# AndreiBarsan/DynSLAM

Measured on AMD Instinct MI355X. Metric: frames/sec TSDF integrate+raycast (KITTI 1242x375, 5mm voxels); HBM GB/s vs peak, higher is better.
Workload: dtype f32; 1 GPU; configs[1]: static map only, synthetic KITTI-like street 1242x375, preset 5mm (voxel 0.005 m, mu 0.02 m), frames 5..2062 of a 2063-frame sequence, one volume per GPU; visible_blocks_last_frame=122661, allocated_blocks=8388608, status=3, decay=False, swap=False, instances=0

## Files before the change

dynslam_amd/csrc/dsr_engine.hip:

```cpp
#include <sched.h>

#include "dsr_internal.h"
#include "dsr_math.h"
using namespace dsr_internal;
#include "k_alloc.h"
#include "k_composite.h"
#include "k_decay.h"
#include "k_integrate.h"
#include "k_raycast.h"
#include "k_swap.h"
#include "k_small.h"
#include "k_batch.h"
#include "k_batch_gc.h"
#include "../../include/dsr_track.h"
#include "../../include/dsr_gc.h"

extern "C" {
int dsri_batch_flush(dsr_batch *b);
bool dsri_batch_is_live(dsr_batch *b);
void dsri_batch_drop_deferred(dsr_batch *b);
}

namespace dsr_internal {
std::atomic<int> g_enginesOnDevice[64];
// ... 122 lines not shown
  F(e->scene.swapState); F(e->scene.swapStored); F(e->swapStagingDev); F(e->swapIdsDev); F(e->swapFlagsDev);
  F(e->scene.swapSlot); F(e->scene.hostSlabs);
  if (e->hostUsedSeen) (void)hipHostFree(e->hostUsedSeen);
  if (e->hostUsedEvent) (void)hipEventDestroy(e->hostUsedEvent);
  for (auto p : e->hostSlabs) (void)hipHostFree(p);
  for (int k = 0; k < 2; ++k) {
    if (e->upPin[k]) (void)hipHostFree(e->upPin[k]);
    if (e->upSlotFree[k]) (void)hipEventDestroy(e->upSlotFree[k]);
  }
  F(e->upDev); F(e->pvDev); F(e->xferRgb); F(e->xferDepth);
  F(e->rgbAlt); F(e->depthAlt);
  for (hipEvent_t ev : {e->evAltFree, e->evFusionRead}) if (ev) (void)hipEventDestroy(ev);
  if (e->viewStream && e->ownsViewStream) (void)hipStreamDestroy(e->viewStream);
  if (e->pvPin) (void)hipHostFree(e->pvPin);
  if (e->statusHost) (void)hipHostFree(e->statusHost);
  for (hipEvent_t ev : {e->evUploaded, e->evIngested, e->evView, e->evViewRead}) if (ev) (void)hipEventDestroy(ev);
  if (e->xEvent) (void)hipEventDestroy(e->xEvent);
  if (e->xEvent2) (void)hipEventDestroy(e->xEvent2);
  if (e->orderEvent) (void)hipEventDestroy(e->orderEvent);
  for (auto &p : e->profPending) { (void)hipEventDestroy(p.a); (void)hipEventDestroy(p.b); }
  for (auto ev : e->eventPool) (void)hipEventDestroy(ev);
  if (e->evList) (void)hipEventDestroy(e->evList);
  if (e->evExpected) (void)hipEventDestroy(e->evExpected);
  if (e->sideStream) (void)hipStreamDestroy(e->sideStream);
  if (e->stream && e->ownsStream) (void)hipStreamDestroy(e->stream);
}

int expected_depths(dsr_engine *e, RenderStateDev &rs, const FrameP &p);

int allocate_scene(dsr_engine *e) {
  e->sceneVersion++;
  e->noVisibleValid = false;
  e->listVersion++;
  float proj[4]; depth_proj(e, proj);
  FrameP p = make_frame_params(e, e->M_d, e->invM_d, proj);
  RenderStateDev &rs = e->live;
  { int st = before_fusion(e); if (st) return st; }
  if (e->sidePending) { HIP_TRY(hipStreamWaitEvent(e->stream, e->evExpected, 0)); e->sidePending = false; }
  if (e->smallPath) {
    const int tx0 = e->viewBox[0] / 16, ty0 = e->viewBox[1] / 16;
    const int tx1 = div_up(std::min(e->viewBox[2], e->W), 16), ty1 = div_up(std::min(e->viewBox[3], e->H), 16);
    if (tx1 > tx0 && ty1 > ty0)
      LAUNCH(e, "alloc_mark", k_alloc_mark<true>, dim3(tx1 - tx0, ty1 - ty0), dim3(256), p, e->scene, (const float *)e->depth,
             rs.visType, tx0, ty0);
    if (e->statusDev) e->statusSeq++;
    {
      ProfScope _ps(e, "small_alloc_visible");
      hipLaunchKernelGGL(k_small_alloc_visible, dim3(1), dim3(kSmallThreads), e->smallLdsBytes, e->stream, p, e->scene,
                         (const float *)e->depth, rs.visType, e->numTilesE, e->allocWork, rs.visibleIDs, rs.visBlocks, e->noBlocks,
                         e->statusDev, e->statusSeq, reinterpret_cast<int2 *>(rs.minmax), rs.rayBox, e->smallLists ? 1 : 0);
    }
    HIP_TRY(hipGetLastError());
    { int st = after_fusion(e); if (st) return st; }
    e->liveExp.valid = true; e->liveExp.onSide = false; e->liveExp.version = e->listVersion; e->liveExp.M = e->M_d;
    memcpy(e->liveExp.proj, proj, sizeof proj);
    return DSR_OK;
  }
  LAUNCH(e, "retest_prev_visible", k_retest_previous_visible, dim3(1024), dim3(256), p, e->scene,
         (const int4 *)rs.visBlocks, rs.visType);
  int2 *allocTile = reinterpret_cast<int2 *>(e->scene.allocTile);
  LAUNCH(e, "alloc_mark", k_alloc_mark<false>, dim3(div_up(e->W, 16), div_up(e->H, 16)), dim3(256), p, e->scene,
         (const float *)e->depth, rs.visType, 0, 0);
  LAUNCH(e, "scan_tiles", k_scan_tile_sums, dim3(1), dim3(1024), allocTile, e->numTilesE, e->scene, (int)SCAN_ALLOC, 0);
  LAUNCH(e, "alloc_commit", k_alloc_commit, dim3(e->numTilesE), dim3(kTileThreads), p, e->scene, allocTile, e->allocWork);
  LAUNCH(e, "alloc_apply", k_alloc_apply, dim3(256), dim3(256), p, e->scene, (const float *)e->depth,
         (const int4 *)e->allocWork, rs.visType);
  LAUNCH(e, "visible_count", k_visible_count<false>, dim3(e->numTilesE), dim3(kTileThreads), p, e->scene, rs.visType, e->tileSums);
  LAUNCH(e, "scan_tiles", k_scan_tile_sums, dim3(1), dim3(1024), e->tileSums, e->numTilesE, e->scene,
         (int)SCAN_VISIBLE_LIVE, e->noBlocks);
  if (e->statusDev) e->statusSeq++;
  LAUNCH(e, "visible_write", k_visible_write, dim3(e->numTilesE), dim3(kTileThreads), e->E, (const uint8_t *)rs.visType,
         (const int2 *)e->tileSums, rs.visibleIDs, e->noBlocks, e->scene, (int)e->s.use_swapping, rs.visBlocks, e->statusDev,
         e->statusSeq);
  HIP_TRY(hipGetLastError());
  { int st = after_fusion(e); if (st) return st; }
  e->liveExp.valid = false;
  if (e->overlapExpected && (e->device >= 64 || g_enginesOnDevice[e->device].load(std::memory_order_relaxed) <= 1)) {
    HIP_TRY(hipEventRecord(e->evList, e->stream));
    HIP_TRY(hipStreamWaitEvent(e->sideStream, e->evList, 0));
    {
      StreamSwap sw(e, e->sideStream);
      int st = expected_depths(e, rs, p);
      if (st) return st;
    }
    HIP_TRY(hipEventRecord(e->evExpected, e->sideStream));
    e->sidePending = true;
    e->liveExp.valid = true; e->liveExp.onSide = true; e->liveExp.version = e->listVersion; e->liveExp.M = e->M_d;
// ... 56 lines not shown
bool pair_render_default() {
  static const bool on = !(getenv("DSR_PAIR_RENDER") && atoi(getenv("DSR_PAIR_RENDER")) == 0);
  return on;
}
int launch_icp_maps(dsr_engine *e, const FrameP &p) {
  RenderStateDev &rs = e->live;
  dim3 g(div_up(e->W, 16), div_up(e->H, 16));
  if (rs.rayBox) LAUNCH(e, "icp_maps", k_icp_maps_box, g, dim3(256), p, e->scene, (const float4 *)rs.raycastResult, e->pointsMap,
                        e->normalsMap, rs.raycastImage, (const int32_t *)rs.rayBox);
  else LAUNCH(e, "icp_maps", k_icp_maps, g, dim3(256), p, e->scene, (const float4 *)rs.raycastResult, e->pointsMap,
              e->normalsMap, rs.raycastImage);
  return DSR_OK;
}
int flush_track_render(dsr_engine *e) {
  if (!e->trackRender.pending) return DSR_OK;
  e->trackRender.pending = false;
  int st = launch_raycast(e, "raycast", e->trackRender.p, e->live);
  if (st) return st;
  if ((st = launch_icp_maps(e, e->trackRender.p))) return st;
  HIP_TRY(hipGetLastError());
  return DSR_OK;
}

const char *status_text(int status) {
  return status == DSR_E_OUT_OF_BLOCKS ? "out of voxel blocks / excess list entries"
                                       : "allocation ray longer than the order key allows: the pose is not rigid (k_alloc.h)";
}

int sticky_status(dsr_engine *e, int *status) {
  static_assert(CTR_NO_VISIBLE_LIVE + 2 == CTR_STATUS, "the three words are fetched with one copy");
  int32_t w[3] = {0, 0, 0};
  HIP_TRY(hipMemcpyAsync(w, e->scene.ctr + CTR_NO_VISIBLE_LIVE, sizeof w, hipMemcpyDeviceToHost, e->stream));
  HIP_TRY(hipStreamSynchronize(e->stream));
  *status = w[2];
  e->noVisibleSeen = w[0]; e->noVisibleValid = true;
  return DSR_OK;
}

int published_status(dsr_engine *e, int *status) {
  if (!e->statusHost) return sticky_status(e, status);
  const int seq = e->statusSeq;
  for (unsigned spins = 1;; ++spins) {
    if ((int)((unsigned)__atomic_load_n(e->statusHost + 2, __ATOMIC_ACQUIRE) - (unsigned)seq) >= 0) break;
    if ((spins & 0xfff) == 0) {
      const hipError_t q = hipStreamQuery(e->stream);
      if (q == hipSuccess) {
// ... 75 lines not shown
  LAUNCH(e, "scan_tiles", k_scan_tile_sums, dim3(1), dim3(1024), e->tileSums, e->numTilesE, e->scene, (int)SCAN_SWAP_OUT,
         (int)kTransferBlocks);
  LAUNCH(e, "swap_list", (k_swap_write<true>), dim3(e->numTilesE), dim3(kTileThreads), e->scene, e->E,
         (const uint8_t *)e->live.visType, (const int2 *)e->tileSums, e->swapIdsDev, e->swapFlagsDev);
  LAUNCH(e, "swapout_move", k_swapout_move, dim3(1024), dim3(256), e->scene, (const int32_t *)e->swapIdsDev);
  e->hostUsedUpper += kTransferBlocks;
  e->hostUsedCallsSince++;
  if (!e->hostUsedPending) {
    HIP_TRY(hipMemcpyAsync(e->hostUsedSeen, e->scene.ctr + CTR_HOST_USED, 4, hipMemcpyDeviceToHost, e->stream));
    HIP_TRY(hipEventRecord(e->hostUsedEvent, e->stream));
    e->hostUsedPending = true;
    e->hostUsedCallsSince = 0;
  }
  HIP_TRY(hipGetLastError());
  return DSR_OK;
}

}

std::string &dsr_internal::last_error() {
  thread_local std::string message;
  return message;
}
int dsr_internal::engine_set_device(dsr_engine *e) { return set_device(e); }
void dsr_internal::prof_resolve_pending(dsr_engine *e) { prof_resolve(e); }
int dsr_internal::engine_flush_deferred(dsr_engine *e) {
  int st = flush_track_render(e);
  if (st) return st;
  if (e->ownerBatch) {
    if (dsri_batch_is_live(e->ownerBatch)) return dsri_batch_flush(e->ownerBatch);
    e->ownerBatch = nullptr;
  }
  return DSR_OK;
}
void dsr_internal::engine_prof_resolve(dsr_engine *e) { prof_resolve(e); }
int dsr_internal::engine_reset(dsr_engine *e) { return reset_scene(e); }
void dsr_internal::engine_list_entries(dsr_engine *e, const char *label, bool owning, const SceneP &sc, int2 *tileSums, int32_t *out,
                                       int capacity, int lengthCtr) {
  const int scanMode = lengthCtr == CTR_NO_ALLOCATED ? SCAN_ALLOCATED : SCAN_NCAND;
  if (owning) LAUNCH(e, label, k_owning_count, dim3(e->numTilesE), dim3(kTileThreads), sc, e->E, tileSums);
  else LAUNCH(e, label, k_allocated_count, dim3(e->numTilesE), dim3(kTileThreads), sc, e->E, tileSums);
  LAUNCH(e, "scan_tiles", k_scan_tile_sums, dim3(1), dim3(1024), tileSums, e->numTilesE, sc, scanMode, capacity);
  if (owning) LAUNCH(e, label, k_owning_write, dim3(e->numTilesE), dim3(kTileThreads), sc, e->E, (const int2 *)tileSums, out, capacity);
  else LAUNCH(e, label, k_allocated_write, dim3(e->numTilesE), dim3(kTileThreads), sc, e->E, (const int2 *)tileSums, out, capacity);
}
void dsr_internal::engine_scan_counts(dsr_engine *e, const SceneP &sc, const uint32_t *counts, const int32_t *nPtr, int n, int2 *tileSums,
                                      uint32_t *offsets) {
// ... 89 lines not shown

  int st = set_device(e);
  if (st) { delete e; return st; }
#define ALLOC(expr) if ((st = (expr)) != DSR_OK) { free_all(e); delete e; return st; }
  if (s.view_pipeline < DSR_VIEW_PIPELINE_AUTO || s.view_pipeline > DSR_VIEW_PIPELINE_SHARED) { delete e; return fail(DSR_E_ARG, "bad view_pipeline"); }
  const int pvMode = s.view_pipeline == DSR_VIEW_PIPELINE_OFF ? 0 : s.view_pipeline == DSR_VIEW_PIPELINE_PER_ENGINE ? 1
                     : s.view_pipeline == DSR_VIEW_PIPELINE_SHARED ? 3
                     : getenv("DSR_PIPELINED_VIEW") ? atoi(getenv("DSR_PIPELINED_VIEW")) : (s.sync_status ? 3 : 0);
  auto shared_stream = [&](hipStream_t *table) -> hipStream_t {
    if (e->device < 0 || e->device >= 64) return nullptr;
    std::lock_guard<std::mutex> lock(g_ioMutex);
    if (!table[e->device] && create_stream(&table[e->device]) != hipSuccess) table[e->device] = nullptr;
    return table[e->device];
  };
  if (pvMode == 3 && s.sdf_local_block_num <= 16384 && (e->stream = shared_stream(g_sharedViewStream))) e->ownsStream = false;
  else if (pvMode >= 2 && s.sdf_local_block_num <= 16384 && (e->stream = shared_stream(g_sharedSmallStream))) e->ownsStream = false;
  else if (create_stream(&e->stream) != hipSuccess) { delete e; return fail(DSR_E_DEVICE, "hipStreamCreate failed"); }
  e->overlapExpected = s.sdf_local_block_num >= (1 << 20);
  if (const char *ov = getenv("DSR_OVERLAP_EXPECTED")) e->overlapExpected = atoi(ov) != 0;
  if (e->overlapExpected &&
      (hipStreamCreateWithFlags(&e->sideStream, hipStreamNonBlocking) != hipSuccess ||
       hipEventCreateWithFlags(&e->evList, order_event_flags()) != hipSuccess ||
       hipEventCreateWithFlags(&e->evExpected, order_event_flags()) != hipSuccess)) { free_all(e); delete e; return fail(DSR_E_DEVICE, "side stream creation failed"); }
  ALLOC(dmalloc(&e->scene.table, (size_t)e->E));
  ALLOC(dmalloc(&e->scene.vba, (size_t)e->noBlocks * kBlockBytes));
  ALLOC(dmalloc(&e->scene.voxelAllocList, (size_t)e->noBlocks));
  ALLOC(dmalloc(&e->scene.excessAllocList, (size_t)e->noExcess));
  ALLOC(dmalloc(&e->scene.ctr, (size_t)CTR_COUNT));
  ALLOC(dmalloc(&e->scene.work, (size_t)WORK_COUNT));
  ALLOC(dmalloc(&e->scene.allocKey, (size_t)e->E));
  ALLOC(dmalloc(&e->scene.allocGrp, (size_t)e->numTilesE * (kTile / 32)));
  ALLOC(dmalloc(&e->scene.allocTile, (size_t)e->numTilesE + 1));
  {
    const int cells = ((e->W + 7) / 8) * ((e->H + 7) / 8);
    e->smallPath = e->smallVolume && !s.use_swapping && e->E <= kSmallMaxEntries && e->E % 8 == 0 && e->numTilesE <= kSmallMaxTiles &&
                   small_lds_bytes(cells) <= 64 * 1024;
    if (e->smallPath) {
      ALLOC(dmalloc(&e->scene.visGrp, (size_t)kSmallBitWords * 4));
      ALLOC(dmalloc(&e->scene.visBits, (size_t)kSmallBitWords));
      ALLOC(dmalloc(&e->scene.allocBits, (size_t)kSmallBitWords));
      ALLOC(dmalloc(&e->scene.allocIds, (size_t)e->noBlocks));
      e->smallLdsBytes = small_lds_bytes(cells);
      const size_t withLists = std::max(e->smallLdsBytes, sizeof(SmallShared) + small_lists_lds_bytes(e->noBlocks));
      e->smallLists = withLists <= 64 * 1024 && !(getenv("DSR_SMALL_LISTS") && atoi(getenv("DSR_SMALL_LISTS")) == 0);
      if (e->smallLists) e->smallLdsBytes = withLists;
      e->pairRender = pair_render_default();
// ... 182 lines not shown
  Mat4 M; memcpy(M.m, m, sizeof M.m);
  Mat4 inv;
  if (!m4_inv(M, inv)) return fail(DSR_E_ARG, "singular pose");
  e->M_d = M; e->invM_d = inv;
  return DSR_OK;
}
int dsr_get_pose(dsr_engine *e, float m_out[16], float inv_m_out[16]) {
  if (!e) return fail(DSR_E_ARG, "null");
  if (m_out) memcpy(m_out, e->M_d.m, sizeof e->M_d.m);
  if (inv_m_out) memcpy(inv_m_out, e->invM_d.m, sizeof e->invM_d.m);
  return DSR_OK;
}


int dsr_set_fusion_weight_params(dsr_engine *e, int depth_weighting) {
  if (!e) return fail(DSR_E_ARG, "null");
  e->depthWeighting = depth_weighting ? 1 : 0;
  return DSR_OK;
}

int dsr_allocate_scene_from_depth(dsr_engine *e) {
  CHECK_E(e);
  if (!e->hasView) return fail(DSR_E_NO_VIEW, "no view yet");
  int st = allocate_scene(e);
  if (st) return st;
  if (e->s.sync_status) {
    int status = DSR_OK;
    st = published_status(e, &status);
    if (st) return st;
    if (status != DSR_OK) return fail(status, status_text(status));
  }
  return DSR_OK;
}

int dsr_integrate_into_scene(dsr_engine *e) {
  CHECK_E(e);
  if (!e->hasView) return fail(DSR_E_NO_VIEW, "no view yet");
  return integrate_scene(e);
}

int dsr_process_frame(dsr_engine *e) {
  CHECK_E(e);
  if (!e->hasView) return fail(DSR_E_NO_VIEW, "no view yet");
  int st = allocate_scene(e);
  if (st) return st;
  st = integrate_scene(e);
  if (st) return st;
  if (e->s.use_swapping) {
    if ((st = swap_in(e))) return st;
    if ((st = swap_out(e))) return st;
  }
  e->framesProcessed++;
  if (e->s.sync_status) {
    int status = DSR_OK;
    st = published_status(e, &status);
    if (st) return st;
    if (status != DSR_OK) {
      (void)hipMemsetAsync(e->scene.ctr + CTR_STATUS, 0, 4, e->stream);
      if (e->statusHost) e->statusHost[1] = DSR_OK;
      return fail(status, status_text(status));
    }
  }
  return DSR_OK;
}

int dsr_prepare(dsr_engine *e) {
  CHECK_E(e);
  if (!e->hasView) return fail(DSR_E_NO_VIEW, "no view yet");
  float proj[4]; depth_proj(e, proj);
  FrameP p = make_frame_params(e, e->M_d, e->invM_d, proj);
  RenderStateDev &rs = e->live;
  if (e->liveExp.valid && e->liveExp.version == e->listVersion && memcmp(e->liveExp.M.m, e->M_d.m, sizeof e->M_d.m) == 0 &&
      memcmp(e->liveExp.proj, proj, sizeof proj) == 0) {
    if (e->liveExp.onSide) {
      HIP_TRY(hipStreamWaitEvent(e->stream, e->evExpected, 0));
      e->sidePending = false;
    }
  } else {
    if (e->sidePending) { HIP_TRY(hipStreamWaitEvent(e->stream, e->evExpected, 0)); e->sidePending = false; }
    e->liveExp.valid = false;
    int st = expected_depths(e, rs, p);
    if (st) return st;
  }
  if (e->pairRender && rs.rayBox) {
    e->trackRender.pending = true;
    e->trackRender.p = p;
    HIP_TRY(hipGetLastError());
    return DSR_OK;
  }
  {
// ... 201 lines not shown
                  float *depth_out) {
  CHECK_E_NOFLUSH(e);
  return render_common(e, type, pose_m, intrinsics, rgba_out, depth_out, false);
}

int dsr_get_image_dev(dsr_engine *e, int type, const float pose_m[16], const float intrinsics[4], void *rgba_out_dev,
                      void *depth_out_dev) {
  CHECK_E_NOFLUSH(e);
  return render_common(e, type, pose_m, intrinsics, rgba_out_dev, depth_out_dev, true);
}

int dsr_engine_share_stream(dsr_engine *e, dsr_engine *owner) {
  CHECK_E(e);
  if (!owner || owner == e) return fail(DSR_E_ARG, "bad stream owner");
  if (owner->device != e->device) return fail(DSR_E_ARG, "engines on different GPUs cannot share a stream");
  if (e->pipelinedView || owner->pipelinedView) return fail(DSR_E_ARG, "not with pipelined views (they have streams of their own)");
  HIP_TRY(hipStreamSynchronize(e->stream));
  if (e->sideStream) HIP_TRY(hipStreamSynchronize(e->sideStream));
  if (e->ownsStream && e->stream) (void)hipStreamDestroy(e->stream);
  e->stream = owner->stream;
  e->ownsStream = false;
  e->borrowedStream = true;
  e->overlapExpected = false;
  e->liveExp.valid = false;
  return DSR_OK;
}


struct dsr_batch {
  dsr_engine *source = nullptr;
  int device = 0;
  std::vector<dsr_engine *> vols;
  std::vector<BatchVolP> volsHost;
  BatchVolP *volsDev = nullptr;
  bool pair = false, pendingTrack = false;
  BatchFrames liveFrames;
  BatchFrameP *freeTableDev = nullptr;
  BatchTrackerDev *tracker = nullptr;
};
namespace {
std::mutex g_batchMutex;
std::vector<dsr_batch *> g_liveBatches;
}
bool dsri_batch_is_live(dsr_batch *b) {
  std::lock_guard<std::mutex> lock(g_batchMutex);
  return std::find(g_liveBatches.begin(), g_liveBatches.end(), b) != g_liveBatches.end();
// ... 373 lines not shown

int dsr_gc_debug_alloc_list(dsr_engine *e, int32_t *ids_out, int32_t capacity, int32_t *n, int32_t *valid) {
  CHECK_E(e);
  if (!n || !valid || capacity < 0 || (capacity > 0 && !ids_out)) return fail(DSR_E_ARG, "bad arguments");
  if (!e->scene.allocIds || !e->smallLists) return fail(DSR_E_ARG, "this engine keeps no sorted list of allocated entries");
  int32_t c[2] = {0, 0};
  HIP_TRY(hipMemcpyAsync(c, e->scene.ctr + CTR_NO_ALLOC_IDS, sizeof c, hipMemcpyDeviceToHost, e->stream));
  HIP_TRY(hipStreamSynchronize(e->stream));
  *n = c[0]; *valid = c[1];
  const int m = std::min(std::min(c[0], capacity), e->noBlocks);
  if (m > 0) {
    HIP_TRY(hipMemcpyAsync(ids_out, e->scene.allocIds, (size_t)m * 4, hipMemcpyDeviceToHost, e->stream));
    HIP_TRY(hipStreamSynchronize(e->stream));
  }
  return DSR_OK;
}

int dsr_gc_debug_fifo(dsr_engine *e, int32_t out[3]) {
  if (!e || !out) return fail(DSR_E_ARG, "bad arguments");
  out[0] = e->fifoHead; out[1] = e->fifoLen; out[2] = e->fifoCap;
  return DSR_OK;
}

int dsr_dump_swap_state(dsr_engine *e, uint8_t *states, uint8_t *has_stored) {
  CHECK_E(e);
  if (!e->scene.swapState) return fail(DSR_E_ARG, "swapping is not enabled");
  if (states) HIP_TRY(hipMemcpyAsync(states, e->scene.swapState, (size_t)e->E, hipMemcpyDeviceToHost, e->stream));
  if (has_stored) HIP_TRY(hipMemcpyAsync(has_stored, e->scene.swapStored, (size_t)e->E, hipMemcpyDeviceToHost, e->stream));
  HIP_TRY(hipStreamSynchronize(e->stream));
  return DSR_OK;
}

int dsr_dump_stored_block(dsr_engine *e, int entry, dsr_voxel *out, int *present) {
  CHECK_E(e);
  if (!present || entry < 0 || entry >= e->E) return fail(DSR_E_ARG, "bad entry");
  *present = 0;
  if (!e->scene.swapState) return DSR_OK;
  uint8_t flag = 0;
  HIP_TRY(hipMemcpy(&flag, e->scene.swapStored + entry, 1, hipMemcpyDeviceToHost));
  if (!flag) return DSR_OK;
  HIP_TRY(hipStreamSynchronize(e->stream));
  int32_t slot = -1;
  HIP_TRY(hipMemcpy(&slot, e->scene.swapSlot + entry, 4, hipMemcpyDeviceToHost));
  if (slot < 0 || slot >= (long long)e->hostSlabs.size() * e->scene.slabBlocks) return fail(DSR_E_DEVICE, "host store inconsistent");
  *present = 1;
  if (out) {
// ... 149 lines not shown
```

dynslam_amd/csrc/dsr_internal.h:

```cpp
#pragma once
#include <hip/hip_runtime.h>

#include <algorithm>
#include <atomic>
#include <cmath>
#include <cstdio>
#include <cstdlib>
#include <cstring>
#include <map>
#include <mutex>
#include <new>
#include <string>
#include <unordered_map>
#include <vector>

#include "dsr_device.h"
#include "dsr_insert.h"
#include "../../include/dsr_mesh.h"
#include "../../include/dsr_track.h"

using namespace dsr;

struct dsr_dense_grid;
struct dsr_erase_params;
// ... 20 lines not shown
struct RenderStateDev {
  int32_t *visibleIDs = nullptr;
  int32_t *visibleIDsAlt = nullptr;
  int4 *visBlocks = nullptr;
  int4 *visBlocksAlt = nullptr;
  uint8_t *visType = nullptr;
  float2 *minmax = nullptr;
  float4 *raycastResult = nullptr;
  uchar4 *raycastImage = nullptr;
  int32_t *rayBox = nullptr;
  int ctrIdx = CTR_NO_VISIBLE_LIVE;
};

struct ProfRec { std::string name; double ms = 0; long long launches = 0; };

struct dsr_engine {
  dsr_settings s;
  dsr_calib calib;
  int device = 0;
  hipStream_t stream = nullptr;
  hipStream_t sideStream = nullptr;
  hipEvent_t evList = nullptr, evExpected = nullptr;
  bool overlapExpected = true;
  unsigned long long listVersion = 0;
  struct { bool valid = false; bool onSide = false; unsigned long long version = 0; Mat4 M; float proj[4] = {0, 0, 0, 0}; } liveExp;
  int W = 0, H = 0, Wr = 0, Hr = 0, P = 0;
  int noBuckets = 0, noExcess = 0, E = 0, noBlocks = 0;
  int numTilesE = 0, numTilesB = 0, numTilesMax = 0;
  uint32_t maxSteps = 0;
  int gridPersistent = 2048;
  int gridDecay = 2048;
  int gridIntegrate = 8192;
  bool smallVolume = false;
  bool smallPath = false;
  bool smallLists = false;
  size_t smallLdsBytes = 0;
  int viewBox[4] = {0, 0, 0, 0};
  int blankBox[4] = {0, 0, 0, 0};
  bool blankValid = false;
  int gridExpected = 128;
  Mat4 calibInv, M_d, invM_d;

  SceneP scene{};
  RenderStateDev live, freeview;
  int2 *tileSums = nullptr;
  uint2 *integrateStats = nullptr;
// ... 150 lines not shown
extern std::mutex g_ioMutex;
extern hipStream_t g_ioStream[64];
hipError_t create_stream(hipStream_t *out);
int io_stream(dsr_engine *e, hipStream_t *out);
unsigned order_event_flags();
int make_event(hipEvent_t *ev, bool hostWaits = false);
int before_view_write(dsr_engine *e, hipStream_t stream);
int view_written(dsr_engine *e, hipStream_t stream);
int begin_view_modify(dsr_engine *e);
int before_fusion(dsr_engine *e);
int after_fusion(dsr_engine *e);
hipStream_t vstream(dsr_engine *e);
void cutout_write_region(const dsr_engine *instance, bool direct, int x0, int y0, int w, int h, int wr[4]);
void cutout_written(dsr_engine *instance, bool direct, int x0, int y0, int w, int h);
void tracker_free(dsr_engine *e);
struct BatchTrackerDev;
int batch_track_check(const dsr_track_settings *settings);
int batch_track(dsr_engine *src, dsr_engine *const *vols, int n, const dsr_track_settings *settings, BatchTrackerDev **bt,
                dsr_track_result *out);
void batch_tracker_free(BatchTrackerDev *bt);
extern std::atomic<int> g_enginesOnDevice[64];
int engine_set_device(dsr_engine *e);
int engine_flush_deferred(dsr_engine *e);
void engine_prof_resolve(dsr_engine *e);
void engine_list_entries(dsr_engine *e, const char *label, bool owning, const SceneP &sc, int2 *tileSums, int32_t *out, int capacity,
                         int lengthCtr = CTR_DECAY_NCAND);
void engine_free_flagged(dsr_engine *e, const int32_t *cand, const int32_t *nCandPtr);
void engine_scan_counts(dsr_engine *e, const SceneP &sc, const uint32_t *counts, const int32_t *nPtr, int n, int2 *tileSums,
                        uint32_t *offsets);
int engine_reset(dsr_engine *e);
int engine_ensure_fifo(dsr_engine *e, int slots);
int engine_add_host_slab(dsr_engine *e);
int engine_small_bit_words();
bool engine_in_live_batch(dsr_engine *e);
int engine_render(dsr_engine *e, int type, const float pose_m[16], const float intrinsics[4], void *rgba_out, void *depth_out,
                  bool outIsDevice);
int mesh_release(dsr_engine *e);
int dense_grid_check(dsr_engine *e, const dsr_dense_grid *grid, const char *what, bool importFields, dsr::DenseP &g, long long &n);
int erase_mask_check(const dsr_engine *e, const dsr_dense_grid *grid, const void *mask, const dsr_erase_params *params);
bool host_range_pinned(const void *p, size_t bytes);
int short_division_exact(hipStream_t stream, float b, bool *exact);
struct Scratch {
  const char *what;
  std::vector<void *> ptrs;
  hipStream_t stream = nullptr;
  bool ordered = false;
// ... 34 lines not shown
  unsigned long long *keysA, *keysB, *voxels;
  uint32_t *bucketsA, *bucketsB;
  int32_t *info, *exc, *excRank, *consumes, *blockRank, *res, *nUnique;
  int2 *plan;
  uint8_t *tmp;
  size_t tmpBytes = 0;
  explicit InsertScratch(const char *what) : sc(what) {}
  int init(int N, bool withSort, hipStream_t stream);
};
int ordered_insert(dsr_engine *dst, const dsr::MergeP &m, int N, const InsertScratch &s);
int ordered_insert(dsr_engine *dst, int N, const InsertScratch &s);
struct InsertOutcome { int32_t res[MR_COUNT]; unsigned long long voxels; int dropped; };
int insert_read_back(dsr_engine *e, const InsertScratch &s, InsertOutcome &o);
inline int two_volume_check(const dsr_engine *dst, const dsr_engine *src, const float *m, const char *what, const char *mName) {
  const std::string w(what);
  if (!dst || !src || !m) return fail(DSR_E_ARG, w + ": null argument");
  if (dst == src) return fail(DSR_E_ARG, w + ": dst and src are the same engine");
  if (dst->device != src->device) return fail(DSR_E_ARG, w + ": the engines sit on different devices (move one with dsr_snapshot_export / _import)");
  if (dst->s.use_swapping || src->s.use_swapping) return fail(DSR_E_ARG, w + ": engines with use_swapping are not supported");
  if (!rigid_transform(m)) return fail(DSR_E_ARG, w + ": " + mName + " is not a rigid transform");
  return DSR_OK;
}
}
using dsr_internal::host_range_pinned;
using dsr_internal::short_division_exact;

#define LAUNCH(e, name, kernel, grid, block, ...)                                \
  do {                                                                           \
    dsr_internal::ProfScope _ps((e), (name));                                    \
    hipLaunchKernelGGL(kernel, grid, block, 0, (e)->stream, __VA_ARGS__);        \
  } while (0)

#define CHECK_E_NOFLUSH(e)                                  \
  if (!(e)) return fail(DSR_E_ARG, "null engine");          \
  { int _st = dsr_internal::engine_set_device(e); if (_st) return _st; }
#define CHECK_E(e)                                          \
  CHECK_E_NOFLUSH(e)                                        \
  if ((e)->trackRender.pending || (e)->ownerBatch) { int _st = dsr_internal::engine_flush_deferred(e); if (_st) return _st; }
```

dynslam_amd/csrc/dsr_view.hip:

```cpp
#include "dsr_internal.h"
#include "k_edges.h"

using namespace dsr_internal;

namespace dsr_internal {
std::mutex g_ioMutex;
hipStream_t g_ioStream[64] = {};
}

namespace dsr_internal {


hipError_t create_stream(hipStream_t *out) { return hipStreamCreateWithFlags(out, hipStreamNonBlocking); }

int io_stream(dsr_engine *e, hipStream_t *out) {
  if (e->device < 0 || e->device >= 64) return fail(DSR_E_ARG, "device ordinal beyond the I/O stream table");
  std::lock_guard<std::mutex> lock(g_ioMutex);
  if (!g_ioStream[e->device]) HIP_TRY(create_stream(&g_ioStream[e->device]));
  *out = g_ioStream[e->device];
  return DSR_OK;
}

unsigned order_event_flags() { return hipEventDisableTiming | hipEventReleaseToDevice; }
int make_event(hipEvent_t *ev, bool hostWaits) {
// ... 16 lines not shown
  HIP_TRY(hipEventRecord(e->evView, stream));
  e->viewEventValid = true;
  return DSR_OK;
}
int io_reads_view(dsr_engine *e, hipStream_t io) {
  if (!e->viewEventValid) {
    int st = make_event(&e->evView, true);
    if (st) return st;
    HIP_TRY(hipEventRecord(e->evView, e->stream));
    e->viewEventValid = true;
  }
  HIP_TRY(hipStreamWaitEvent(io, e->evView, 0));
  return DSR_OK;
}
int io_read_done(dsr_engine *e, hipStream_t io) {
  int st = make_event(&e->evViewRead, true);
  if (st) return st;
  HIP_TRY(hipEventRecord(e->evViewRead, io));
  e->viewReadEver = true;
  return DSR_OK;
}

hipStream_t vstream(dsr_engine *e) { return e->pipelinedView ? e->viewStream : e->stream; }

void cutout_write_region(const dsr_engine *instance, bool direct, int x0, int y0, int w, int h, int wr[4]) {
  const int W = instance->W, H = instance->H;
  wr[0] = 0; wr[1] = 0; wr[2] = W; wr[3] = H;
  if (!direct || !instance->blankValid) return;
  const int b[4] = {std::max(0, x0), std::max(0, y0), std::min(W, x0 + w), std::min(H, y0 + h)};
  const int *o = instance->blankBox;
  const bool bEmpty = b[0] >= b[2] || b[1] >= b[3], oEmpty = o[0] >= o[2] || o[1] >= o[3];
  if (bEmpty && oEmpty) { wr[2] = 0; wr[3] = 0; return; }
  if (bEmpty) { for (int k = 0; k < 4; ++k) wr[k] = o[k]; return; }
  if (oEmpty) { for (int k = 0; k < 4; ++k) wr[k] = b[k]; return; }
  wr[0] = std::min(b[0], o[0]); wr[1] = std::min(b[1], o[1]); wr[2] = std::max(b[2], o[2]); wr[3] = std::max(b[3], o[3]);
}
void cutout_written(dsr_engine *instance, bool direct, int x0, int y0, int w, int h) {
  instance->blankValid = direct;
  instance->blankBox[0] = std::max(0, x0); instance->blankBox[1] = std::max(0, y0);
  instance->blankBox[2] = std::min(instance->W, x0 + w); instance->blankBox[3] = std::min(instance->H, y0 + h);
}

struct ViewTarget { uchar4 *rgb; float *depth; };

int begin_view_replace(dsr_engine *e, hipStream_t ws, ViewTarget *t) {
  int st = before_view_write(e, ws);
// ... 70 lines not shown
  HIP_TRY(hipStreamWaitEvent(consumer, e->evUploaded, 0));
  *cDev = e->upDev;
  *dDev = e->upDev + e->upDepthOff;
  return DSR_OK;
}
int upload_consumed(dsr_engine *e, hipStream_t consumer) {
  HIP_TRY(hipEventRecord(e->evIngested, consumer));
  e->ingestPending = true;
  return DSR_OK;
}

int filter_view(dsr_engine *e, float *depth) {
  if (!e->s.use_bilateral_filter) return DSR_OK;
  HIP_TRY(hipMemcpyAsync(e->depthTmp, depth, (size_t)e->P * 4, hipMemcpyDeviceToDevice, e->stream));
  dim3 g(div_up(e->W, 16), div_up(e->H, 16));
  for (int k = 0; k < 5; ++k) {
    if (k & 1) LAUNCH(e, "filter_depth", k_filter_depth, g, dim3(256), (const float *)e->depthTmp, depth, e->W, e->H);
    else LAUNCH(e, "filter_depth", k_filter_depth, g, dim3(256), (const float *)depth, e->depthTmp, e->W, e->H);
  }
  HIP_TRY(hipMemcpyAsync(depth, e->depthTmp, (size_t)e->P * 4, hipMemcpyDeviceToDevice, e->stream));
  return DSR_OK;
}

int convert_view(dsr_engine *e, const void *rgbDev, const void *depthDev, bool uploaded = false) {
  const float a = e->calib.disparity_calib[0], b = e->calib.disparity_calib[1];
  const size_t rgbBytes = (size_t)e->Wr * e->Hr * 4;
  hipStream_t ws = vstream(e);
  ViewTarget t;
  int st = begin_view_replace(e, ws, &t);
  if (st) return st;
  {
    StreamSwap sw(e, ws);
    if (((uintptr_t)rgbDev & 15) == 0 && ((uintptr_t)depthDev & 15) == 0) {
      const int nRgbVec = (int)(rgbBytes / 16), nQuads = div_up(e->P, 4);
      LAUNCH(e, "view_ingest", k_view_ingest, dim3(div_up(std::max(nRgbVec, nQuads), 256)), dim3(256), (const uint4 *)rgbDev,
             reinterpret_cast<uint4 *>(t.rgb), nRgbVec, e->Wr * e->Hr, (const short *)depthDev, t.depth, e->P, a, b);
    } else {
      HIP_TRY(hipMemcpyAsync(t.rgb, rgbDev, rgbBytes, hipMemcpyDeviceToDevice, ws));
      HIP_TRY(hipMemcpyAsync(e->rawDepth, depthDev, (size_t)e->P * 2, hipMemcpyDeviceToDevice, ws));
      LAUNCH(e, "depth_to_float", k_depth_to_float, dim3(div_up(div_up(e->P, 4), 256)), dim3(256), e->rawDepth, t.depth,
             e->P, a, b);
    }
    HIP_TRY(hipGetLastError());
    if (uploaded && (st = upload_consumed(e, ws))) return st;
    if ((st = filter_view(e, t.depth))) return st;
  }
  return end_view_replace(e, ws);
}

}
// ... 31 lines not shown
  HIP_TRY(hipGetDevice(&dev));
  if (sc.device != dev) {
    if (sc.in) (void)hipFree(sc.in);
    if (sc.out) (void)hipFree(sc.out);
    sc.in = sc.out = nullptr; sc.inCap = sc.outCap = 0;
    sc.device = dev;
  }
  int st = conv_reserve(&sc.in, &sc.inCap, inBytes);
  if (st) return st;
  if ((st = conv_reserve(&sc.out, &sc.outCap, outBytes))) return st;
  HIP_TRY(hipMemcpy(sc.in, in, inBytes, hipMemcpyHostToDevice));
  st = convert_dev<K, TI, TO>(kernel, -1, nullptr, sc.in, sc.out, n);
  if (st) return st;
  if (hipMemcpy(out, sc.out, outBytes, hipMemcpyDeviceToHost) != hipSuccess) return fail(DSR_E_DEVICE, "conversion copy failed");
  return DSR_OK;
}

}

extern "C" {


int dsr_update_view(dsr_engine *e, const uint8_t *rgba, const int16_t *depth_mm) {
  CHECK_E(e);
  if (!rgba || !depth_mm) return fail(DSR_E_ARG, "null image");
  const uint8_t *cDev = nullptr, *dDev = nullptr;
  int st = upload_frame(e, vstream(e), rgba, (size_t)e->Wr * e->Hr * 4, depth_mm, (size_t)e->P * 2, &cDev, &dDev);
  if (st) return st;
  return convert_view(e, cDev, dDev, true);
}

int dsr_update_view_bgr(dsr_engine *e, const uint8_t *bgr, const int16_t *depth_mm) {
  CHECK_E(e);
  if (!bgr || !depth_mm) return fail(DSR_E_ARG, "null image");
  const uint8_t *cDev = nullptr, *dDev = nullptr;
  hipStream_t ws = vstream(e);
  int st = upload_frame(e, ws, bgr, (size_t)e->Wr * e->Hr * 3, depth_mm, (size_t)e->P * 2, &cDev, &dDev);
  if (st) return st;
  ViewTarget t;
  if ((st = begin_view_replace(e, ws, &t))) return st;
  const float a = e->calib.disparity_calib[0], b = e->calib.disparity_calib[1];
  {
    StreamSwap sw(e, ws);
    if (e->Wr * e->Hr == e->P) {
      LAUNCH(e, "view_ingest", k_view_ingest_bgr, dim3(div_up(div_up(e->P, 4), 256)), dim3(256), (const uint32_t *)cDev,
             reinterpret_cast<uint4 *>(t.rgb), e->P, (const short *)dDev, t.depth, a, b);
    } else {
      LAUNCH(e, "view_ingest", k_bgr_to_rgba, dim3(div_up(e->Wr * e->Hr, 256)), dim3(256), cDev, t.rgb, e->Wr * e->Hr);
      LAUNCH(e, "depth_to_float", k_depth_to_float, dim3(div_up(div_up(e->P, 4), 256)), dim3(256), (const short *)dDev, t.depth, e->P, a, b);
    }
    HIP_TRY(hipGetLastError());
    if ((st = upload_consumed(e, ws)) || (st = filter_view(e, t.depth))) return st;
  }
  return end_view_replace(e, ws);
}

int dsr_update_view_dev(dsr_engine *e, const void *rgba_dev, const void *depth_mm_dev) {
  CHECK_E(e);
  if (!rgba_dev || !depth_mm_dev) return fail(DSR_E_ARG, "null image");
  return convert_view(e, rgba_dev, depth_mm_dev);
}

int dsr_set_view_float(dsr_engine *e, const uint8_t *rgba, const float *depth_m) {
  CHECK_E(e);
  if (!rgba || !depth_m) return fail(DSR_E_ARG, "null image");
  const uint8_t *cDev = nullptr, *dDev = nullptr;
  hipStream_t ws = vstream(e);
  int st = upload_frame(e, ws, rgba, (size_t)e->Wr * e->Hr * 4, depth_m, (size_t)e->P * 4, &cDev, &dDev);
  if (st) return st;
  ViewTarget t;
  if ((st = begin_view_replace(e, ws, &t))) return st;
  {
    StreamSwap sw(e, ws);
    LAUNCH(e, "set_view", k_set_view_ingest, dim3(div_up(std::max(e->Wr * e->Hr, e->P), 256)), dim3(256), (const uchar4 *)cDev, t.rgb,
           e->Wr * e->Hr, (const float *)dDev, t.depth, e->P);
    HIP_TRY(hipGetLastError());
    if ((st = upload_consumed(e, ws))) return st;
  }
  return end_view_replace(e, ws);
}

int dsr_set_view_float_dev(dsr_engine *e, const void *rgba_dev, const void *depth_m_dev) {
  CHECK_E(e);
// ... 140 lines not shown
  static unsigned long long done[64] = {};
  if (from == to || from >= 64 || to >= 64) return DSR_OK;
  std::lock_guard<std::mutex> lock(m);
  if (done[from] & (1ull << to)) return DSR_OK;
  int can = 0;
  if (hipDeviceCanAccessPeer(&can, from, to) == hipSuccess && can) {
    int prev = 0;
    (void)hipGetDevice(&prev);
    if (hipSetDevice(from) == hipSuccess) {
      const hipError_t err = hipDeviceEnablePeerAccess(to, 0);
      if (err != hipSuccess && err != hipErrorPeerAccessAlreadyEnabled) (void)hipGetLastError();
    }
    (void)hipSetDevice(prev);
  }
  done[from] |= 1ull << to;
  return DSR_OK;
}

static int extract_silhouette(dsr_engine *main_engine, dsr_engine *instance, const uint8_t *mask, const uint8_t *maskDev,
                              int x0, int y0, int box_w, int box_h, const uint8_t *rmask = nullptr, const uint8_t *rmaskDev = nullptr,
                              int rx0 = 0, int ry0 = 0, int rbw = 0, int rbh = 0) {
  CHECK_E(main_engine);
  if (!instance || (!mask && !maskDev) || box_w <= 0 || box_h <= 0) return fail(DSR_E_ARG, "bad silhouette arguments");
  const bool blank = rbw > 0 || rbh > 0 || rmask || rmaskDev;
  if (blank && ((!rmask && !rmaskDev) || rbw <= 0 || rbh <= 0)) return fail(DSR_E_ARG, "bad silhouette arguments");
  if (!main_engine->hasView) return fail(DSR_E_NO_VIEW, "no view yet");
  if (instance->W != main_engine->W || instance->H != main_engine->H ||
      instance->Wr != main_engine->Wr || instance->Hr != main_engine->Hr || main_engine->W != main_engine->Wr ||
      main_engine->H != main_engine->Hr)
    return fail(DSR_E_ARG, "main and instance engines must share the image size");
  int maskSlot = -1, rmaskSlot = -1;
  if (!maskDev && blank && !rmaskDev) {
    int st = ensure_mask_ring(main_engine, std::max((size_t)box_w * box_h, (size_t)rbw * rbh));
    if (st) return st;
  }
  if (!maskDev) {
    int st = upload_mask(main_engine, mask, box_w, box_h, &maskDev, &maskSlot);
    if (st) return st;
  }
  if (blank && !rmaskDev) {
    if (rmask == mask && rbw == box_w && rbh == box_h) rmaskDev = maskDev;
    else { int st = upload_mask(main_engine, rmask, rbw, rbh, &rmaskDev, &rmaskSlot); if (st) return st; }
  }
  dsr_engine *e = main_engine;
  const bool forcePeerPath = getenv("DSR_FORCE_PEER_PATH") != nullptr;
  const bool peer = instance->device != e->device || forcePeerPath;
// ... 176 lines not shown
```

Measured before the change: 3687 frames/s.

## Run next frame's view ingest and allocation on side stream early

Adds an early-allocation window. After a frame is integrated, the next frame's view upload/convert and the first allocation kernels (retest visible, alloc_mark, scan, commit) are issued on the side stream, gated on an event recorded after integration. The main stream joins via an event before alloc_apply. The aim is to overlap the previous frame's trailing work (raycast, ICP maps) with the next frame's ingest and allocation, and to hide launch gaps. This adds cross-stream events and state tracking, with a risk of ordering bugs between the side and main streams, and it only turns on for large block pools on a single engine per device.

```diff
diff --git a/dynslam_amd/csrc/dsr_engine.hip b/dynslam_amd/csrc/dsr_engine.hip
--- a/dynslam_amd/csrc/dsr_engine.hip
+++ b/dynslam_amd/csrc/dsr_engine.hip
@@ -168,19 +168,23 @@
   for (auto ev : e->eventPool) (void)hipEventDestroy(ev);
   if (e->evList) (void)hipEventDestroy(e->evList);
   if (e->evExpected) (void)hipEventDestroy(e->evExpected);
+  for (hipEvent_t ev : {e->evIntegrated, e->evCommitted, e->evSideView}) if (ev) (void)hipEventDestroy(ev);
   if (e->sideStream) (void)hipStreamDestroy(e->sideStream);
   if (e->stream && e->ownsStream) (void)hipStreamDestroy(e->stream);
 }
 
 int expected_depths(dsr_engine *e, RenderStateDev &rs, const FrameP &p);
 
-int allocate_scene(dsr_engine *e) {
+int allocate_scene(dsr_engine *e, bool mayEarly) {
   e->sceneVersion++;
   e->noVisibleValid = false;
   e->listVersion++;
   float proj[4]; depth_proj(e, proj);
   FrameP p = make_frame_params(e, e->M_d, e->invM_d, proj);
   RenderStateDev &rs = e->live;
+  const bool early = mayEarly && early_window(e);
+  if (!early) { int st = engine_close_early(e); if (st) return st; }
+  e->earlyOpen = false;
   { int st = before_fusion(e); if (st) return st; }
   if (e->sidePending) { HIP_TRY(hipStreamWaitEvent(e->stream, e->evExpected, 0)); e->sidePending = false; }
   if (e->smallPath) {
@@ -202,13 +206,26 @@
     memcpy(e->liveExp.proj, proj, sizeof proj);
     return DSR_OK;
   }
-  LAUNCH(e, "retest_prev_visible", k_retest_previous_visible, dim3(1024), dim3(256), p, e->scene,
-         (const int4 *)rs.visBlocks, rs.visType);
   int2 *allocTile = reinterpret_cast<int2 *>(e->scene.allocTile);
-  LAUNCH(e, "alloc_mark", k_alloc_mark<false>, dim3(div_up(e->W, 16), div_up(e->H, 16)), dim3(256), p, e->scene,
-         (const float *)e->depth, rs.visType, 0, 0);
-  LAUNCH(e, "scan_tiles", k_scan_tile_sums, dim3(1), dim3(1024), allocTile, e->numTilesE, e->scene, (int)SCAN_ALLOC, 0);
-  LAUNCH(e, "alloc_commit", k_alloc_commit, dim3(e->numTilesE), dim3(kTileThreads), p, e->scene, allocTile, e->allocWork);
+  {
+    if (early) HIP_TRY(hipStreamWaitEvent(e->sideStream, e->evIntegrated, 0));
+    StreamSwap sw(e, early ? e->sideStream : e->stream);
+    if (early) { int st = before_fusion(e); if (st) return st; }
+    LAUNCH(e, "retest_prev_visible", k_retest_previous_visible, dim3(1024), dim3(256), p, e->scene,
+           (const int4 *)rs.visBlocks, rs.visType);
+    LAUNCH(e, "alloc_mark", k_alloc_mark<false>, dim3(div_up(e->W, 16), div_up(e->H, 16)), dim3(256), p, e->scene,
+           (const float *)e->depth, rs.visType, 0, 0);
+    LAUNCH(e, "scan_tiles", k_scan_tile_sums, dim3(1), dim3(1024), allocTile, e->numTilesE, e->scene, (int)SCAN_ALLOC, 0);
+    LAUNCH(e, "alloc_commit", k_alloc_commit, dim3(e->numTilesE), dim3(kTileThreads), p, e->scene, allocTile, e->allocWork);
+  }
+  if (early) {
+    hipEvent_t join = e->earlyViewCopied ? e->evSideView : e->evCommitted;
+    HIP_TRY(hipEventRecord(join, e->sideStream));
+    HIP_TRY(hipStreamWaitEvent(e->stream, join, 0));
+    e->earlyViewOnSide = false;
+    e->earlyViewCopied = false;
+    e->earlyFrames++;
+  }
   LAUNCH(e, "alloc_apply", k_alloc_apply, dim3(256), dim3(256), p, e->scene, (const float *)e->depth,
          (const int4 *)e->allocWork, rs.visType);
   LAUNCH(e, "visible_count", k_visible_count<false>, dim3(e->numTilesE), dim3(kTileThreads), p, e->scene, rs.visType, e->tileSums);
@@ -311,6 +328,13 @@
   return DSR_OK;
 }
 
+int open_early(dsr_engine *e) {
+  if (!early_policy(e)) return DSR_OK;
+  HIP_TRY(hipEventRecord(e->evIntegrated, e->stream));
+  e->earlyOpen = true;
+  return DSR_OK;
+}
+
 const char *status_text(int status) {
   return status == DSR_E_OUT_OF_BLOCKS ? "out of voxel blocks / excess list entries"
                                        : "allocation ray longer than the order key allows: the pose is not rigid (k_alloc.h)";
@@ -432,7 +456,34 @@
   thread_local std::string message;
   return message;
 }
-int dsr_internal::engine_set_device(dsr_engine *e) { return set_device(e); }
+int dsr_internal::engine_set_device(dsr_engine *e) {
+  int st = set_device(e);
+  return st ? st : engine_close_early(e);
+}
+bool dsr_internal::early_policy(const dsr_engine *e) {
+  if (!e->earlyAlloc || !e->sideStream || !e->evIntegrated || e->smallPath || e->s.use_swapping || !e->ownsStream || e->borrowedStream)
+    return false;
+  if (e->earlyAlloc >= 2) return true;
+  return e->noBlocks >= (1 << 20) && (e->device >= 64 || g_enginesOnDevice[e->device].load(std::memory_order_relaxed) <= 1);
+}
+bool dsr_internal::early_window(dsr_engine *e) {
+  if (!early_policy(e)) return false;
+  if (e->earlyOpen) return true;
+  if (hipStreamQuery(e->stream) != hipSuccess) return false;
+  if (hipEventRecord(e->evIntegrated, e->stream) != hipSuccess) return false;
+  e->earlyOpen = true;
+  return true;
+}
+int dsr_internal::engine_close_early(dsr_engine *e) {
+  e->earlyOpen = false;
+  if (e->earlyViewOnSide) {
+    HIP_TRY(hipEventRecord(e->evSideView, e->sideStream));
+    HIP_TRY(hipStreamWaitEvent(e->stream, e->evSideView, 0));
+    e->earlyViewOnSide = false;
+    e->earlyViewCopied = false;
+  }
+  return DSR_OK;
+}
 void dsr_internal::prof_resolve_pending(dsr_engine *e) { prof_resolve(e); }
 int dsr_internal::engine_flush_deferred(dsr_engine *e) {
   int st = flush_track_render(e);
@@ -568,6 +619,15 @@
       (hipStreamCreateWithFlags(&e->sideStream, hipStreamNonBlocking) != hipSuccess ||
        hipEventCreateWithFlags(&e->evList, order_event_flags()) != hipSuccess ||
        hipEventCreateWithFlags(&e->evExpected, order_event_flags()) != hipSuccess)) { free_all(e); delete e; return fail(DSR_E_DEVICE, "side stream creation failed"); }
+  e->earlyAlloc = 1;
+  if (const char *ea = getenv("DSR_EARLY_ALLOC")) e->earlyAlloc = std::max(0, std::min(2, atoi(ea)));
+  if (e->earlyAlloc == 1 && s.sdf_local_block_num < (1 << 20)) e->earlyAlloc = 0;
+  if (s.use_swapping || !e->ownsStream) e->earlyAlloc = 0;
+  if (e->earlyAlloc &&
+      ((!e->sideStream && hipStreamCreateWithFlags(&e->sideStream, hipStreamNonBlocking) != hipSuccess) ||
+       hipEventCreateWithFlags(&e->evIntegrated, order_event_flags()) != hipSuccess ||
+       hipEventCreateWithFlags(&e->evCommitted, order_event_flags()) != hipSuccess ||
+       hipEventCreateWithFlags(&e->evSideView, hipEventDisableTiming) != hipSuccess)) { free_all(e); delete e; return fail(DSR_E_DEVICE, "side stream creation failed"); }
   ALLOC(dmalloc(&e->scene.table, (size_t)e->E));
   ALLOC(dmalloc(&e->scene.vba, (size_t)e->noBlocks * kBlockBytes));
   ALLOC(dmalloc(&e->scene.voxelAllocList, (size_t)e->noBlocks));
@@ -796,7 +856,7 @@
 int dsr_allocate_scene_from_depth(dsr_engine *e) {
   CHECK_E(e);
   if (!e->hasView) return fail(DSR_E_NO_VIEW, "no view yet");
-  int st = allocate_scene(e);
+  int st = allocate_scene(e, false);
   if (st) return st;
   if (e->s.sync_status) {
     int status = DSR_OK;
@@ -814,9 +874,9 @@
 }
 
 int dsr_process_frame(dsr_engine *e) {
-  CHECK_E(e);
+  CHECK_E_FRAME(e);
   if (!e->hasView) return fail(DSR_E_NO_VIEW, "no view yet");
-  int st = allocate_scene(e);
+  int st = allocate_scene(e, true);
   if (st) return st;
   st = integrate_scene(e);
   if (st) return st;
@@ -832,14 +892,15 @@
     if (status != DSR_OK) {
       (void)hipMemsetAsync(e->scene.ctr + CTR_STATUS, 0, 4, e->stream);
       if (e->statusHost) e->statusHost[1] = DSR_OK;
+      (void)open_early(e);
       return fail(status, status_text(status));
     }
   }
-  return DSR_OK;
+  return open_early(e);
 }
 
 int dsr_prepare(dsr_engine *e) {
-  CHECK_E(e);
+  CHECK_E_FRAME(e);
   if (!e->hasView) return fail(DSR_E_NO_VIEW, "no view yet");
   float proj[4]; depth_proj(e, proj);
   FrameP p = make_frame_params(e, e->M_d, e->invM_d, proj);
@@ -1087,6 +1148,7 @@
   e->ownsStream = false;
   e->borrowedStream = true;
   e->overlapExpected = false;
+  e->earlyAlloc = 0;
   e->liveExp.valid = false;
   return DSR_OK;
 }
@@ -1506,6 +1568,12 @@
   return DSR_OK;
 }
 
+int dsr_debug_early_alloc(dsr_engine *e, int64_t out[2]) {
+  if (!e || !out) return fail(DSR_E_ARG, "bad arguments");
+  out[0] = e->earlyFrames; out[1] = e->earlyAlloc;
+  return DSR_OK;
+}
+
 int dsr_dump_swap_state(dsr_engine *e, uint8_t *states, uint8_t *has_stored) {
   CHECK_E(e);
   if (!e->scene.swapState) return fail(DSR_E_ARG, "swapping is not enabled");
diff --git a/dynslam_amd/csrc/dsr_internal.h b/dynslam_amd/csrc/dsr_internal.h
--- a/dynslam_amd/csrc/dsr_internal.h
+++ b/dynslam_amd/csrc/dsr_internal.h
@@ -66,6 +66,12 @@
   hipStream_t sideStream = nullptr;
   hipEvent_t evList = nullptr, evExpected = nullptr;
   bool overlapExpected = true;
+  int earlyAlloc = 0;
+  hipEvent_t evIntegrated = nullptr, evCommitted = nullptr, evSideView = nullptr;
+  bool earlyOpen = false;
+  bool earlyViewOnSide = false;
+  bool earlyViewCopied = false;
+  long long earlyFrames = 0;
   unsigned long long listVersion = 0;
   struct { bool valid = false; bool onSide = false; unsigned long long version = 0; Mat4 M; float proj[4] = {0, 0, 0, 0}; } liveExp;
   int W = 0, H = 0, Wr = 0, Hr = 0, P = 0;
@@ -262,6 +268,9 @@
 extern std::atomic<int> g_enginesOnDevice[64];
 int engine_set_device(dsr_engine *e);
 int engine_flush_deferred(dsr_engine *e);
+bool early_policy(const dsr_engine *e);
+bool early_window(dsr_engine *e);
+int engine_close_early(dsr_engine *e);
 void engine_prof_resolve(dsr_engine *e);
 void engine_list_entries(dsr_engine *e, const char *label, bool owning, const SceneP &sc, int2 *tileSums, int32_t *out, int capacity,
                          int lengthCtr = CTR_DECAY_NCAND);
@@ -342,6 +351,7 @@
   return DSR_OK;
 }
 }
+extern "C" int dsr_debug_early_alloc(dsr_engine *e, int64_t out[2]);
 using dsr_internal::host_range_pinned;
 using dsr_internal::short_division_exact;
 
@@ -357,3 +367,10 @@
 #define CHECK_E(e)                                          \
   CHECK_E_NOFLUSH(e)                                        \
   if ((e)->trackRender.pending || (e)->ownerBatch) { int _st = dsr_internal::engine_flush_deferred(e); if (_st) return _st; }
+#define CHECK_E_FRAME(e)                                    \
+  if (!(e)) return fail(DSR_E_ARG, "null engine");          \
+  { int _st = dsr_internal::set_device(e); if (_st) return _st; } \
+  if ((e)->trackRender.pending || (e)->ownerBatch) {        \
+    int _st = dsr_internal::engine_close_early(e);          \
+    if (_st || (_st = dsr_internal::engine_flush_deferred(e))) return _st; \
+  }
diff --git a/dynslam_amd/csrc/dsr_view.hip b/dynslam_amd/csrc/dsr_view.hip
--- a/dynslam_amd/csrc/dsr_view.hip
+++ b/dynslam_amd/csrc/dsr_view.hip
@@ -62,6 +62,16 @@
 }
 
 hipStream_t vstream(dsr_engine *e) { return e->pipelinedView ? e->viewStream : e->stream; }
+
+int ingest_stream(dsr_engine *e, bool mayUseSide, hipStream_t *ws) {
+  *ws = vstream(e);
+  if (e->pipelinedView) return DSR_OK;
+  if (!mayUseSide || !early_window(e)) return engine_close_early(e);
+  HIP_TRY(hipStreamWaitEvent(e->sideStream, e->evIntegrated, 0));
+  e->earlyViewOnSide = true;
+  *ws = e->sideStream;
+  return DSR_OK;
+}
 
 void cutout_write_region(const dsr_engine *instance, bool direct, int x0, int y0, int w, int h, int wr[4]) {
   const int W = instance->W, H = instance->H;
@@ -178,10 +188,9 @@
   return DSR_OK;
 }
 
-int convert_view(dsr_engine *e, const void *rgbDev, const void *depthDev, bool uploaded = false) {
+int convert_view(dsr_engine *e, const void *rgbDev, const void *depthDev, hipStream_t ws, bool uploaded = false) {
   const float a = e->calib.disparity_calib[0], b = e->calib.disparity_calib[1];
   const size_t rgbBytes = (size_t)e->Wr * e->Hr * 4;
-  hipStream_t ws = vstream(e);
   ViewTarget t;
   int st = begin_view_replace(e, ws, &t);
   if (st) return st;
@@ -259,12 +268,13 @@
 
 
 int dsr_update_view(dsr_engine *e, const uint8_t *rgba, const int16_t *depth_mm) {
-  CHECK_E(e);
-  if (!rgba || !depth_mm) return fail(DSR_E_ARG, "null image");
+  CHECK_E_FRAME(e);
+  if (!rgba || !depth_mm) { (void)engine_close_early(e); return fail(DSR_E_ARG, "null image"); }
   const uint8_t *cDev = nullptr, *dDev = nullptr;
-  int st = upload_frame(e, vstream(e), rgba, (size_t)e->Wr * e->Hr * 4, depth_mm, (size_t)e->P * 2, &cDev, &dDev);
-  if (st) return st;
-  return convert_view(e, cDev, dDev, true);
+  hipStream_t ws = nullptr;
+  int st = ingest_stream(e, !e->s.use_bilateral_filter, &ws);
+  if (st || (st = upload_frame(e, ws, rgba, (size_t)e->Wr * e->Hr * 4, depth_mm, (size_t)e->P * 2, &cDev, &dDev))) return st;
+  return convert_view(e, cDev, dDev, ws, true);
 }
 
 int dsr_update_view_bgr(dsr_engine *e, const uint8_t *bgr, const int16_t *depth_mm) {
@@ -293,9 +303,13 @@
 }
 
 int dsr_update_view_dev(dsr_engine *e, const void *rgba_dev, const void *depth_mm_dev) {
-  CHECK_E(e);
-  if (!rgba_dev || !depth_mm_dev) return fail(DSR_E_ARG, "null image");
-  return convert_view(e, rgba_dev, depth_mm_dev);
+  CHECK_E_FRAME(e);
+  if (!rgba_dev || !depth_mm_dev) { (void)engine_close_early(e); return fail(DSR_E_ARG, "null image"); }
+  hipStream_t ws = nullptr;
+  int st = ingest_stream(e, !e->s.use_bilateral_filter, &ws);
+  if (st) return st;
+  if (e->earlyViewOnSide && ((((uintptr_t)rgba_dev | (uintptr_t)depth_mm_dev) & 15) != 0)) e->earlyViewCopied = true;
+  return convert_view(e, rgba_dev, depth_mm_dev, ws);
 }
 
 int dsr_set_view_float(dsr_engine *e, const uint8_t *rgba, const float *depth_m) {
@@ -482,6 +496,7 @@
                               int rx0 = 0, int ry0 = 0, int rbw = 0, int rbh = 0) {
   CHECK_E(main_engine);
   if (!instance || (!mask && !maskDev) || box_w <= 0 || box_h <= 0) return fail(DSR_E_ARG, "bad silhouette arguments");
+  { int st = engine_close_early(instance); if (st) return st; }
   const bool blank = rbw > 0 || rbh > 0 || rmask || rmaskDev;
   if (blank && ((!rmask && !rmaskDev) || rbw <= 0 || rbh <= 0)) return fail(DSR_E_ARG, "bad silhouette arguments");
   if (!main_engine->hasView) return fail(DSR_E_NO_VIEW, "no view yet");
```

Result: slower. 3626 frames/s (-1.6%).
